# hsiehScalAR/KNODE-Cosserat

Hardware: AMD Instinct MI355X
Metric: rod-steps/sec (N=100 segments, batch=1024) (higher is better)
Workload: dtype f64

## Files before the change

knode-cosserat_amd/csrc/kr_mso_impl.hpp:

```cpp
#pragma once
#include "kr_ms_impl.hpp"

namespace kr {

constexpr int MSO_B0 = 7 + 17 * (MS_P - 1);
#ifndef KR_MSO_LAG
#define KR_MSO_LAG 1
#endif
constexpr int MSO_LAG = KR_MSO_LAG;
#ifndef KR_MSO_TRIP_WAITS
#define KR_MSO_TRIP_WAITS 1
#endif
#ifndef KR_MSO_TRIP_CARRY
#define KR_MSO_TRIP_CARRY 0
#endif
static_assert(MSO_B0 + MS_P <= WAVE, "the verifying lanes must fit beside the forward-difference lanes");

template <typename T, int HS>
__host__ __device__ inline size_t mso_lds_elems(int N) {
  return ms_lds_elems<T, HS>(N, true, false) + 80;
}

__device__ __forceinline__ void wave_sync_lds() {
  __builtin_amdgcn_fence(__ATOMIC_ACQ_REL, "wavefront");
  __builtin_amdgcn_wave_barrier();
}

#define KR_LDS __attribute__((address_space(3)))
#define KR_SCHED_ALL_BUT_DS 0x047f
template <typename T, int NV>
__device__ __forceinline__ void lds_load_vec(const T* src, T (&v)[NV]) {
  using V = typename Vec16<T>::type;
  constexpr int n = Vec16<T>::n;
  static_assert(NV % n == 0, "vector load needs a multiple of 16 bytes");
  const KR_LDS V* s = (const KR_LDS V*)src;
#pragma unroll
  for (int c = 0; c < NV / n; ++c) {
    const V x = s[c];
#pragma unroll
    for (int e = 0; e < n; ++e) v[c * n + e] = x[e];
  }
}
template <typename T, int NV>
__device__ __forceinline__ void lds_store_vec(T* dst, const T (&v)[NV]) {
  using V = typename Vec16<T>::type;
  constexpr int n = Vec16<T>::n;
  static_assert(NV % n == 0, "vector store needs a multiple of 16 bytes");
  KR_LDS V* d = (KR_LDS V*)dst;
#pragma unroll
  for (int c = 0; c < NV / n; ++c) {
    V x;
#pragma unroll
    for (int e = 0; e < n; ++e) x[e] = v[c * n + e];
    d[c] = x;
  }
}

template <typename T>
struct LeadTile {
  using V = typename Vec16<T>::type;
  static constexpr int NT = 12 / Vec16<T>::n;
  V t[NT];
};
template <typename T>
__device__ __forceinline__ void lds_load_lead(const T* src, LeadTile<T>& x) {
  using V = typename Vec16<T>::type;
  const KR_LDS V* s = (const KR_LDS V*)src;
#pragma unroll
  for (int c = 0; c < LeadTile<T>::NT; ++c) x.t[c] = s[c];
}
__device__ __forceinline__ void lead_pin(LeadTile<double>& x) {
  asm volatile("" : "+v"(x.t[0]), "+v"(x.t[1]), "+v"(x.t[2]), "+v"(x.t[3]), "+v"(x.t[4]), "+v"(x.t[5]));
}
template <typename T>
__device__ __forceinline__ void lead_unpack(const LeadTile<T>& x, T (&v)[12]) {
  constexpr int n = Vec16<T>::n;
#pragma unroll
  for (int c = 0; c < LeadTile<T>::NT; ++c) {
#pragma unroll
    for (int e = 0; e < n; ++e) v[c * n + e] = x.t[c][e];
  }
}

template <typename U>
__device__ __forceinline__ U own_sgpr(U v) {
  asm volatile("" : "+s"(v));
  return v;
}

template <typename U>
__device__ __forceinline__ U* own_sgpr_global(U* p) {
  uintptr_t v = (uintptr_t)p;
  asm volatile("" : "+s"(v));
  return (U*)(__attribute__((address_space(1))) U*)v;
}

template <typename T>
__device__ __forceinline__ T quad_pick(int kp, T v0, T v1, T v2, T v3) {
  T v = v3;
  v = kp == 2 ? v2 : v;
  v = kp == 1 ? v1 : v;
  v = kp == 0 ? v0 : v;
  return v;
}

template <int K>
__device__ __forceinline__ void wave_sum_f64_staged(double (&v)[K]) {
  auto stage = [&](auto ctrl) {
    double o[K];
#pragma unroll
    for (int k = 0; k < K; ++k) o[k] = quad_xor<decltype(ctrl)::value>(v[k]);
#pragma unroll
    for (int k = 0; k < K; ++k) v[k] += o[k];
  };
  stage(std::integral_constant<int, 0xB1>{});
  stage(std::integral_constant<int, 0x4E>{});
  stage(std::integral_constant<int, 0x141>{});
  stage(std::integral_constant<int, 0x140>{});
  int lo[K], hi[K];
  double s[K];
#pragma unroll
  for (int k = 0; k < K; ++k) {
    const long long b = __double_as_longlong(v[k]);
    lo[k] = (int)(b & 0xFFFFFFFFll);
    hi[k] = (int)(b >> 32);
    s[k] = 0.0;
  }
#pragma unroll
  for (int r = 0; r < 4; ++r) {
#pragma unroll
    for (int k = 0; k < K; ++k) {
      const int l = __builtin_amdgcn_readlane(lo[k], 16 * r), h = __builtin_amdgcn_readlane(hi[k], 16 * r);
      s[k] += __longlong_as_double(((long long)h << 32) | (unsigned int)l);
    }
  }
#pragma unroll
  for (int k = 0; k < K; ++k) v[k] = s[k];
}

template <typename T, int NC>
__device__ __forceinline__ void mso_pred_update(MsPred<T, NC>& Q, int order, int predictor, int lane, const T* Xs,
                                                MsStamps& stamps) {
  if (!__builtin_amdgcn_readfirstlane((int)(order == MS_ORDER_LP && Q.lp_good))) {
    ms_pred_update<T>(Q, order, KR_ST_CONVERGED, predictor, lane, Xs, stamps);
    return;
  }
#ifdef KR_MS_STAMPS
  unsigned long long tpu;
  KR_STAMP(tpu);
#endif
  float err_lp = 0.f;
  if (Q.lp_have) {
#pragma unroll
    for (int q = 0; q < MS_EPL; ++q) {
      const int e = lane + q * WAVE;
      if (e < MS_NE) {
        const double x = (double)Xs[e];
        double b[NC];
        lp_basis<T, NC>(Q.Hx[q], b);
        err_lp = fmaxf(err_lp, update_ratio(x - lp_eval<NC>(Q.lpa, b), x));
      }
    }
  }
  const float em_lp = wave_max_nonneg(err_lp);
#ifdef KR_MS_STAMPS
  KR_STAMP_ADD(stamps.a1, tpu);
#endif
  const bool lp_tested = Q.lp_have;
  const bool keep_fit = lp_tested && em_lp < 1.0e-3f && Q.lp_age < 3;
  Q.lp_age = keep_fit ? Q.lp_age + 1 : 0;
  Q.lp_have = keep_fit;
  if (!keep_fit && predictor >= MS_ORDER_LP && Q.avail >= NC - 1) {
    double Sn[lp_nsum<NC>()];
#pragma unroll
    for (int k = 0; k < lp_nsum<NC>(); ++k) Sn[k] = 0.0;
#pragma unroll
    for (int q = 0; q < MS_EPL; ++q) {
      const int e = lane + q * WAVE;
      if (e < MS_NE) {
        const double x = (double)Xs[e];
        double b[NC];
        lp_basis<T, NC>(Q.Hx[q], b);
        const double w = (double)__builtin_amdgcn_rcpf(fmaxf(fabsf((float)x), 1.0f));
        lp_accumulate<NC>(Sn, b, x, w);
      }
    }
    if constexpr (sizeof(T) == 8) {
      wave_sum_f64_staged(Sn);
    } else {
#pragma unroll
      for (int k = 0; k < lp_nsum<NC>(); ++k) Sn[k] = wave_sum_f64(Sn[k]);
    }
    double a[NC];
    if (lp_solve<NC>(Sn, a)) {
#pragma unroll
      for (int k = 0; k < NC; ++k) Q.lpa[k] = a[k];
      Q.lp_have = true;
    }
  }
#ifdef KR_MS_STAMPS
  KR_STAMP_ADD(stamps.a2, tpu);
#endif
  Q.next_order = Q.avail < predictor ? Q.avail : (predictor < MS_HLEV ? predictor : MS_HLEV - 1);
  Q.lp_good = lp_tested && Q.lp_have && em_lp < 1.0e-3f;
  if (lp_tested && Q.lp_have && (em_lp < 3.0e38f || Q.lp_good)) Q.next_order = MS_ORDER_LP;
#ifdef KR_MS_STAMPS
  stamps.osum += (unsigned long long)order; stamps.olast = order;
  for (int p = 0; p < MS_HLEV; ++p) stamps.em[p] = 3.0e38f;
  KR_STAMP_ADD(stamps.a3, tpu);
#endif
#pragma unroll
  for (int q = 0; q < MS_EPL; ++q) {
    const int e = lane + q * WAVE;
#pragma unroll
    for (int k = MS_HLEV - 1; k > 0; --k) Q.Hx[q][k] = Q.Hx[q][k - 1];
    if (e < MS_NE) Q.Hx[q][0] = Xs[e];
  }
  if (Q.avail < MS_HLEV - 1) ++Q.avail;
}

#ifdef KR_MS_STAMPS
struct MsoStats { unsigned long long total = 0, sweeps = 0, merged = 0, quick = 0, chord = 0, rejects = 0, retries = 0, rebuilds = 0, t_sweep = 0, t_alg = 0, t_pred = 0, t_verdict = 0, t_cond = 0, t_fin = 0, t_upd = 0, t_v1 = 0, t_v2 = 0, t_c1 = 0, t_c2 = 0, t_copy = 0; };
#endif

template <typename T, bool DIAG, int HS, int OCC = 1, typename PSRC = RodConst<T>>
__global__ __launch_bounds__(WAVE * MS_WPB, OCC) void mso_sim_kernel(const PSRC Pa, const SimArgs<T> A) {
  extern __shared__ __attribute__((aligned(16))) unsigned char smem_raw[];
  const int N = rod_src_N<T>(Pa);
  const int lane = threadIdx.x & (WAVE - 1);
  const int wv = threadIdx.x / WAVE;
  const int64_t rod = (int64_t)blockIdx.x * MS_WPB + wv;
  if (rod >= A.B) return;
  const auto& Pc = rod_src_row<T>(Pa, rod);
  const size_t rod_elems = (size_t)N * KR_SLOTS;
  T* const a_states = own_sgpr_global(A.states);
  const int64_t a_slot_elems = own_sgpr(A.slot_elems);
  const int a_ring = own_sgpr(A.ring);
  T* const a_tip = own_sgpr_global(A.tip);
  int32_t* const a_status = own_sgpr_global(A.status);
  const int a_residual_test = own_sgpr(A.residual_test), a_predictor = own_sgpr(A.predictor);
  const T hc1 = own_sgpr(A.hc1), hc2 = own_sgpr(A.hc2);
  const int T_steps = own_sgpr((int)A.T_steps);
  using KPSRC = rod_src_keypoints<T, PSRC>;
  constexpr bool KP = KPSRC::value;
  constexpr bool TRIM = OCC == 1 && sizeof(T) == 8 && MSO_LAG == 1;
  const unsigned long long kp_lo = KPSRC::lo(Pa), kp_hi = KPSRC::hi(Pa);
  const MsLds<T> L = ms_carve<T, HS>(reinterpret_cast<T*>(smem_raw) + (size_t)wv * mso_lds_elems<T, HS>(N), N, true, false);
  T* const Es = L.Es;
  T* const XB = L.XB;
  T* const Tm = L.Tm;
  T* const X0 = L.Xs;
  const ptrdiff_t X_d = (L.c12 + (size_t)N * 12) - L.Xs;
  int xsel = 0;
  T* Xs = X0;
  T* XsB = X0 + X_d;
  T* const EsB = Es + MSO_B0 * MS_YP;
  const MsRole R = ms_role(lane, N);
  const int iv = R.iv, col = R.col;
  const bool isA = lane < MSO_B0;
  const bool isB = lane >= MSO_B0 && lane < MSO_B0 + MS_P;
  const int ib = isB ? lane - MSO_B0 : 0;
  const int s_l = isB ? ms_interval_start(ib, R.sbase, R.srem) : R.s_i;
  const int len_l = isB ? R.sbase + (ib < R.srem ? 1 : 0) : R.len_i;
  unsigned kp_marks = 0;
  int kp_rank0 = 0;
  if constexpr (KP) {
    kp_marks = keypoint_window(kp_lo, kp_hi, s_l);
    kp_rank0 = keypoint_rank(kp_lo, kp_hi, s_l);
  }
  ms_cold_fill<T>(rod_src_mem<T>(Pa, rod), L.cold, lane);
  wave_sync();

  auto slot_ptr = [&](int slot) -> T* { return a_states + (int64_t)slot * a_slot_elems + rod * rod_elems; };
  auto state_ptr = [&](int k) -> T* { return slot_ptr(a_ring ? k % 3 : k); };
  T* const lead0 = L.c12;
  const ptrdiff_t lead_d = L.hist - L.c12;
  auto lead_of = [&](int t) -> T* { return lead0 + (ptrdiff_t)(t & 1) * lead_d; };
  auto rebuild = [&](int t) {
    const T* cur = state_ptr(t);
    const T* prv = t > 0 ? state_ptr(t - 1) : (A.prev_init ? A.prev_init + rod * rod_elems : cur);
    T* const lc = lead_of(t);
    T* const lp = lead_of(t - 1);
    for (int j = lane; j < N; j += WAVE) {
      T cv[12], pv[12];
      load_hist_vec<T, 12>(cur + (size_t)j * KR_SLOTS, cv);
      load_hist_vec<T, 12>(prv + (size_t)j * KR_SLOTS, pv);
      lds_store_vec<T, 12>(lc + (size_t)j * 12, cv);
      lds_store_vec<T, 12>(lp + (size_t)j * 12, pv);
    }
    wave_sync();
  };
  using WSRC = rod_src_step_slots<T, PSRC>;
  constexpr int W0 = WSRC::first, WN = WSRC::count;
  constexpr bool LOADS = WN > 0;
  static_assert(!LOADS || (W0 + WN == CD_TDIRS && (W0 == CD_FTIP || W0 == CD_P0)), "the per-step slots end with F_tip, M_tip");
  static_assert(!LOADS || (HS >= 18 && (2 * MS_P + 1) * (HS - 12) >= WN), "the second set lives behind the odd tile in the record area");
  const ptrdiff_t wr_d = LOADS ? (L.hist + (size_t)N * 12) - (L.cold + W0) : 0;
  auto cold_of = [&](int t) -> const T* {
    if constexpr (LOADS) return L.cold + (ptrdiff_t)(t & 1) * wr_d;
    else return L.cold;
  };
  auto base_of = [&](int t) -> const T* {
    if constexpr (LOADS && W0 < CD_FTIP) return L.cold + (ptrdiff_t)(t & 1) * wr_d;
    else return L.cold;
  };
  const T* wrench = nullptr;
  if constexpr (LOADS) wrench = WSRC::hist(Pa) + rod * A.T_steps * WN;
  const T* ctl = A.ctl + rod * A.T_steps * 4;
  auto load_fc = [&](int t) -> V3<T> {
    V3<T> tf{T(0), T(0), T(0)};
#pragma unroll
    for (int k = 0; k < 4; ++k) {
      const T tt = ctl[(size_t)t * 4 + k];
      tf.x += tt * L.cold[CD_TDIRS + k * 3 + 0];
      tf.y += tt * L.cold[CD_TDIRS + k * 3 + 1];
      tf.z += tt * L.cold[CD_TDIRS + k * 3 + 2];
    }
    return {L.cold[CD_RHOAG] + tf.x, L.cold[CD_RHOAG + 1] + tf.y, L.cold[CD_RHOAG + 2] + tf.z};
  };

  const T* s0 = state_ptr(0);
  const T* sp0 = A.prev_init ? A.prev_init + rod * rod_elems : s0;
  MsPred<T> Q;
  double* img = A.pred_io ? A.pred_io + (size_t)rod * MS_PRED_ROWS * WAVE : nullptr;
  if (img && A.pred_load) ms_pred_load<T>(Q, img, lane);
  else ms_pred_init<T>(Q, lane, R, s0, sp0, A.prev_init != nullptr, a_predictor);
  V3<T> vlast, ulast;
  {
    const T* cl = s0 + (size_t)(N - 1) * KR_SLOTS;
    vlast = {cl[SL_V], cl[SL_V + 1], cl[SL_V + 2]};
    ulast = {cl[SL_U], cl[SL_U + 1], cl[SL_U + 2]};
  }
  const T tol = own_sgpr(A.tol), tolA = own_sgpr(A.tolA), fd_eps = own_sgpr(A.fd_eps);
  const int maxit = own_sgpr(A.maxit);
  T kappa = Q.kappa;
  T Gguess = lane < 6 ? A.G[rod * 6 + lane] : T(0);
  MsStamps stamps;
#ifdef KR_MS_STAMPS
  MsoStats st;
  unsigned long long t_begin, tq;
  KR_STAMP(t_begin);
  tq = t_begin;
#endif

  rebuild(0);

  int tA = 0;
  int rsA = 0;
  bool merged = false;
  int it = 0;
  int order = Q.next_order;
  bool retried = false;
  T dn_prev = T(-1);
  bool have_fac = false, below = false;
  float amp = -1.f;
  T dnB = T(-1);
  float ampB = -1.f;
  bool belowB = false;
  int itB = 0, orderB = 0;
  bool pred_skip = false;
  bool reverify = false;
  int resume_at = T_steps;
  T Xreg[MS_P - 1][2];
#pragma unroll
  for (int g = 0; g < MS_P - 1; ++g) Xreg[g][0] = Xreg[g][1] = T(0);
  V3<T> fcA = load_fc(0), fcB = fcA;
  V3<T> fcN = load_fc(T_steps > 1 ? 1 : 0);
  T wN = T(0);
  if constexpr (LOADS) {
    if (lane < WN) {
      L.cold[W0 + lane] = wrench[lane];
      wN = wrench[(size_t)(T_steps > 1 ? 1 : 0) * WN + lane];
    }
    if constexpr (W0 < CD_FTIP) wave_sync_lds();
  }
  static_assert(DIAG, "the in-sweep history record assumes diagonal material matrices");
  T hk_a[3], hk_b[3], hk_c[3];
#pragma unroll
  for (int c = 0; c < 3; ++c) {
    hk_a[c] = L.cold[CD_KSEI + 4 * c] * L.cold[CD_KSEV + c];
    hk_b[c] = -L.cold[CD_KSEI + 4 * c] * L.cold[CD_BSE + 4 * c];
    hk_c[c] = -L.cold[CD_KBTI + 4 * c] * L.cold[CD_BBT + 4 * c];
  }

  ms_pred_guess<T>(Q, order, lane, base_of(0), Xs);
  wave_sync_lds();
  if (order <= 0 && lane < 6) Xs[0 * MS_YP + 7 + lane] = Gguess;
  wave_sync_lds();

  struct Upd { T newPG, newY[MS_P - 1]; };

  while (true) {
    const bool runA = tA < T_steps;
    const int tB = tA - 1;
    T yr[19];
    {
      const T* src = isB ? XsB + ib * MS_YP : Xs + iv * MS_YP;
#pragma unroll
      for (int q = 0; q < 19; ++q) yr[q] = src[q];
    }
    const T hstep = (isA && col > 0) ? fd_eps * fmax(fabs(Xs[iv * MS_YP + (R.comp > 0 ? R.comp : 3)]), T(1)) : T(1);
    int comp = R.comp;
    asm volatile("" : "+v"(comp));
#pragma unroll
    for (int q = 3; q < 19; ++q) yr[q] += q == comp ? hstep : T(0);
    RodState<T> y = rows_to_state(yr);
    const V3<T> fc = isB ? fcB : fcA;
    const int lag = (isA && merged) ? MSO_LAG : 0;
    const bool act = isB ? merged : (isA && runA);
    const int trips = R.lmax + ((merged && runA) ? MSO_LAG : 0);
    T* const out_rod = slot_ptr(rsA);
    T* const kp_out = KPSRC::at(Pa, tB, A.B, rod);
    auto point_of = [&](int k) -> int {
      const int kk = k - lag;
      return s_l + (kk < 0 ? 0 : (kk < len_l ? kk : len_l - 1));
    };
    const T* const lead_n = lead_of(isB ? tB : tA);
    const T* const lead_o = lead_of(isB ? tB + 1 : tB);
    auto hist_older = [&](const T (&lb)[12], T (&pb)[12]) __attribute__((always_inline)) {
#pragma unroll
      for (int c = 0; c < 12; ++c) pb[c] = hc2 * lb[c];
    };
    auto hist_newest = [&](const T (&la)[12], const T (&pb)[12]) __attribute__((always_inline)) -> RodHist<T> {
      T raw[12];
#pragma unroll
      for (int c = 0; c < 12; ++c) raw[c] = fma(hc1, la[c], pb[c]);
      RodHist<T> h;
      h.qh = {raw[0], raw[1], raw[2]};
      h.wh = {raw[3], raw[4], raw[5]};
      h.vh = {raw[6], raw[7], raw[8]};
      h.uh = {raw[9], raw[10], raw[11]};
      h.av = {hk_b[0] * raw[6] + hk_a[0], hk_b[1] * raw[7] + hk_a[1], hk_b[2] * raw[8] + hk_a[2]};
      h.au = {hk_c[0] * raw[9], hk_c[1] * raw[10], hk_c[2] * raw[11]};
      return h;
    };
    auto hist_form = [&](const T (&la)[12], const T (&lb)[12]) __attribute__((always_inline)) -> RodHist<T> {
      T pb[12];
      hist_older(lb, pb);
      return hist_newest(la, pb);
    };
    auto hist_at = [&](int j) __attribute__((always_inline)) -> RodHist<T> {
      T la[12], lb[12];
      lds_load_vec<T, 12>(lead_n + (size_t)j * 12, la);
      lds_load_vec<T, 12>(lead_o + (size_t)j * 12, lb);
      return hist_form(la, lb);
    };
    RodHist<T> hst = hist_at(point_of(0));
    const bool lean = a_ring && tB + 4 <= T_steps;
    if (!merged) {
      auto fd_point = [&](int j, T dsl) __attribute__((always_inline)) {
        RodState<T> k1;
        V3<T> v, u;
        ode_eval<T, DIAG>(Pc, y, hst, fc, k1, v, u);
        hst = hist_at(j + 1);
        y = state_axpy(y, dsl, k1);
      };
#pragma unroll 2
      for (int t = 0; t < R.sbase; ++t) fd_point(R.s_i + t, Pc.ds);
      if (R.srem) fd_point(R.s_i + (R.len_i > R.sbase ? R.sbase : R.sbase - 1), R.len_i > R.sbase ? Pc.ds : T(0));
    } else {
      T* const lead_w = lead_of(tB + 1);
#if KR_MSO_TRIP_CARRY
      T rs = rot_scale(y.h0, y.h1, y.h2, y.h3);
#endif
      auto trip = [&](int k, auto full_tag, auto lean_tag) __attribute__((always_inline)) {
        constexpr int FORM = decltype(full_tag)::value;
        constexpr bool FULL = FORM == 1;
        constexpr bool FIRST = TRIM && FORM == 2;
        constexpr bool LEAN = decltype(lean_tag)::value;
        const int kk = k - lag;
        const bool live = FIRST ? isB : FULL ? act : (act && kk >= 0 && kk < len_l);
        const int j = FIRST ? s_l : FULL ? s_l + kk : point_of(k);
        const int eo = j * 12;
        const int en = FIRST ? (s_l + ((isB && len_l > 1) ? 1 : 0)) * 12 : FULL ? eo + 12 : point_of(k + 1) * 12;
        T la[12], lb[12], pb[12];
#ifdef KR_MSO_PROBE_EARLY_READS
        constexpr bool TUPLES = false;
#else
        constexpr bool TUPLES = KR_MSO_TRIP_WAITS && MSO_LAG < 2 && OCC == 1 && sizeof(T) == 8;
#endif
        LeadTile<T> ta, tb;
        if constexpr (TUPLES) {
          lds_load_lead<T>(lead_o + en, tb);
          __builtin_amdgcn_sched_barrier(KR_SCHED_ALL_BUT_DS);
        } else if constexpr (MSO_LAG >= 2) {
          lds_load_vec<T, 12>(lead_n + en, la);
          lds_load_vec<T, 12>(lead_o + en, lb);
        } else {
          lds_load_vec<T, 12>(lead_o + en, lb);
#ifdef KR_MSO_PROBE_EARLY_READS
          if constexpr (FULL) lds_load_vec<T, 12>(lead_n + en, la);
#endif
        }
        RodState<T> k1;
        V3<T> v, u;
#if KR_MSO_TRIP_CARRY
        ode_eval_s<T, DIAG>(Pc, y, hst, fc, k1, v, u, rs);
#else
        ode_eval<T, DIAG>(Pc, y, hst, fc, k1, v, u);
#endif
        if constexpr (MSO_LAG >= 2) {
          hst = hist_form(la, lb);
          asm volatile("" : "+v"(hst.qh.x), "+v"(hst.qh.y), "+v"(hst.qh.z), "+v"(hst.wh.x), "+v"(hst.wh.y), "+v"(hst.wh.z));
          asm volatile("" : "+v"(hst.vh.x), "+v"(hst.vh.y), "+v"(hst.vh.z), "+v"(hst.uh.x), "+v"(hst.uh.y), "+v"(hst.uh.z));
          asm volatile("" : "+v"(hst.av.x), "+v"(hst.av.y), "+v"(hst.av.z), "+v"(hst.au.x), "+v"(hst.au.y), "+v"(hst.au.z));
        } else {
          if constexpr (TUPLES) {
            asm volatile("" ::"v"(v.x), "v"(v.y), "v"(v.z), "v"(u.x), "v"(u.y), "v"(u.z));
            lead_pin(tb);
            lead_unpack<T>(tb, lb);
          }
          hist_older(lb, pb);
          asm volatile("" : "+v"(pb[0]), "+v"(pb[1]), "+v"(pb[2]), "+v"(pb[3]), "+v"(pb[4]), "+v"(pb[5]), "+v"(pb[6]), "+v"(pb[7]),
                            "+v"(pb[8]), "+v"(pb[9]), "+v"(pb[10]), "+v"(pb[11]));
        }
        if (isB && live) {
          T rec[KR_SLOTS];
          record_from(y, v, u, rec);
          T lead[12];
#pragma unroll
          for (int c = 0; c < 12; ++c) lead[c] = rec[c];
          if constexpr (FULL) {
            if constexpr (!LEAN) {
              T rest[KR_SLOTS - 12];
#pragma unroll
              for (int c = 0; c < KR_SLOTS - 12; ++c) rest[c] = rec[12 + c];
              store_vec<T, KR_SLOTS - 12>(out_rod + (size_t)j * KR_SLOTS + 12, rest);
            }
          } else {
            if (!(lean && k >= R.sbase)) store_record(out_rod + (size_t)j * KR_SLOTS, rec);
          }
          if constexpr (KP) store_keypoint_window(kp_out, kp_marks, kp_rank0, kk, rec);
#ifdef KR_MSO_PROBE_NO_TILE_STORES
          if constexpr (!FULL)
#endif
#ifdef KR_MSO_PROBE_ONE_TILE_STORE
          if constexpr (FULL) {
            T l2[Vec16<T>::n];
#pragma unroll
            for (int c = 0; c < Vec16<T>::n; ++c) l2[c] = lead[c];
            lds_store_vec<T, Vec16<T>::n>(lead_w + eo, l2);
          } else
#endif
          lds_store_vec<T, 12>(lead_w + eo, lead);
        }
        if constexpr (MSO_LAG < 2) {
#ifdef KR_MSO_PROBE_EARLY_READS
          if constexpr (!FULL)
#endif
          {
            if constexpr (TUPLES) lds_load_lead<T>(lead_n + en, ta);
            else lds_load_vec<T, 12>(lead_n + en, la);
          }
          if constexpr (OCC == 1) __builtin_amdgcn_sched_barrier(0);
        }
        const T dsl = live ? Pc.ds : T(0);
        y = state_axpy(y, dsl, k1);
        if constexpr (MSO_LAG < 2) {
          asm volatile("" : "+v"(pb[0]), "+v"(pb[1]), "+v"(pb[2]), "+v"(pb[3]), "+v"(pb[4]), "+v"(pb[5]), "+v"(pb[6]), "+v"(pb[7]),
                            "+v"(pb[8]), "+v"(pb[9]), "+v"(pb[10]), "+v"(pb[11]), "+v"(y.p.z), "+v"(y.h3), "+v"(y.n.z), "+v"(y.m.z),
                            "+v"(y.q.z), "+v"(y.w.z));
#if KR_MSO_TRIP_CARRY
          rs = rot_scale(y.h0, y.h1, y.h2, y.h3);
#endif
          if constexpr (TUPLES) {
            lead_pin(ta);
            lead_unpack<T>(ta, la);
          }
          hst = hist_newest(la, pb);
        }
      };
      int k = 0;
      for (; k < MSO_LAG && k < trips; ++k) trip(k, std::integral_constant<int, 2>{}, std::false_type{});
      auto full_trips = [&](auto lean_tag) __attribute__((always_inline)) {
        for (; k + 1 < R.sbase; k += 2) {
          trip(k, std::true_type{}, lean_tag);
          trip(k + 1, std::true_type{}, lean_tag);
        }
        if (k < R.sbase) {
          trip(k, std::true_type{}, lean_tag);
          ++k;
        }
      };
      if (lean) full_trips(std::true_type{});
      else full_trips(std::false_type{});
      const bool own_final = TRIM && runA;
      for (; k < trips - (own_final ? 1 : 0); ++k) trip(k, std::false_type{}, std::false_type{});
      if (own_final) {
        const bool live = isA && R.lmax - 1 < len_l;
        RodState<T> k1;
        V3<T> v, u;
        ode_eval<T, DIAG>(Pc, y, hst, fc, k1, v, u);
        const T dsl = live ? Pc.ds : T(0);
        y = state_axpy(y, dsl, k1);
      }
    }
#ifdef KR_MS_STAMPS
    KR_STAMP_ADD(st.t_sweep, tq);
    st.sweeps += 1;
    if (merged) st.merged += 1;
#endif

    int ln = lane;
    asm volatile("" : "+v"(ln));
    const int kp = ln & 3;
    const int r = 3 + (ln >> 2);
    const bool plane = ln < 3 * (MS_P - 1);
    const int pi = plane ? ln / 3 : 0;
    const int prow = plane ? ln - 3 * pi : 0;
    const bool glane = ln >= WAVE - 6;
    T er[19];
    state_to_rows(y, er);
    T d[6];
    T updY[MS_P - 1];
    T* dYb = XB;
    float dnf = 0.f;
    bool finite = true;
    Upd U;

    auto finish = [&](const T* X, auto base_slot) -> float {
      T* sp = Tm;
      if (kp == 0) {
#pragma unroll
        for (int g = 1; g < MS_P - 1; ++g) dYb[g * MS_YP + r] = updY[g - 1];
      }
      wave_sync_lds();
      if (plane) {
        const bool p0 = pi == 0;
        const int l0 = p0 ? 0 : 7 + 17 * (pi - 1);
        const int drow = p0 ? 1 : pi;
        T s = Es[base_slot(pi) * MS_YP + prow] - X[(pi + 1) * MS_YP + prow];
        T av[16], dv[16];
#pragma unroll
        for (int c = 0; c < 16; ++c) {
          av[c] = Es[(l0 + 1 + c) * MS_YP + prow];
          dv[c] = dYb[drow * MS_YP + 3 + c];
        }
        __builtin_amdgcn_sched_barrier(0);
        T s2 = T(0);
#pragma unroll
        for (int c = 0; c < 6; c += 2) {
          s = fma(av[c], p0 ? d[c] : dv[c], s);
          s2 = fma(av[c + 1], p0 ? d[c + 1] : dv[c + 1], s2);
        }
        const T s_6 = s, s2_6 = s2;
#pragma unroll
        for (int c = 6; c < 16; c += 2) {
          s = fma(av[c], dv[c], s);
          s2 = fma(av[c + 1], dv[c + 1], s2);
        }
        s = p0 ? s_6 : s;
        s2 = p0 ? s2_6 : s2;
        sp[pi * 3 + prow] = s + s2;
      }
      wave_sync_lds();
      const T xp = X[(pi + 1) * MS_YP + prow];
      T up = T(0);
#pragma unroll
      for (int i = 0; i < MS_P - 1; ++i) {
        const T t = sp[i * 3 + prow];
        up += i <= pi ? t : T(0);
      }
      const int kg = glane ? ln - (WAVE - 6) : 0;
      const T xg = X[0 * MS_YP + 7 + kg];
      T ug = d[5];
      asm volatile("" : "+v"(ug));
      ug = kg == 4 ? d[4] : ug;
      ug = kg == 3 ? d[3] : ug;
      asm volatile("" : "+v"(ug));
      ug = kg == 2 ? d[2] : ug;
      ug = kg == 1 ? d[1] : ug;
      asm volatile("" : "+v"(ug));
      ug = kg == 0 ? d[0] : ug;
      const T newP = xp + up, newG = xg + ug;
      U.newPG = plane ? newP : newG;
      float np = update_ratio(up, xp), ng = update_ratio(ug, xg);
      asm volatile("" : "+v"(np), "+v"(ng));
      unsigned nb = plane ? __float_as_uint(np) : (glane ? __float_as_uint(ng) : 0u);
#pragma unroll
      for (int g = 1; g < MS_P; ++g) {
        const T xy = X[g * MS_YP + r];
        float ny = update_ratio(updY[g - 1], xy);
        U.newY[g - 1] = xy + updY[g - 1];
        asm volatile("" : "+v"(ny));
        nb = max(nb, ((g - 1) & 3) == kp ? __float_as_uint(ny) : 0u);
      }
      const float nf = __uint_as_float(nb);
      return wave_max_nonneg(nf);
    };
    auto apply = [&](T* X) {
      int la = ln;
      asm volatile("" : "+v"(la));
      const bool pl = la < 3 * (MS_P - 1), gl = la >= WAVE - 6;
      const int pa = pl ? la / 3 : 0;
      if (pl || gl) X[pl ? (pa + 1) * MS_YP + (la - 3 * pa) : 0 * MS_YP + 7 + (la - (WAVE - 6))] = U.newPG;
#pragma unroll
      for (int g = 1; g < MS_P; ++g)
        if (g - 1 == (la & 3)) X[g * MS_YP + r] = U.newY[g - 1];
    };

    const bool es_stored = merged;
    if (merged) {
      if (isB || (isA && col == 0)) {
#pragma unroll
        for (int q = 0; q < 19; ++q) Es[ln * MS_YP + q] = er[q];
      }
      if (isB) {
        if (ib == MS_P - 1) {
          T rec[KR_SLOTS];
          record_from(y, vlast, ulast, rec);
          if (!lean) store_record(out_rod + (size_t)(N - 1) * KR_SLOTS, rec);
          if constexpr (KP) store_keypoint(kp_out, kp_lo, kp_hi, N - 1, rec);
          T lead[12];
#pragma unroll
          for (int c = 0; c < 12; ++c) lead[c] = rec[c];
          lds_store_vec<T, 12>(lead_of(tB + 1) + (size_t)(N - 1) * 12, lead);
          if (a_tip) {
            T* tp = a_tip + (rod * T_steps + tB) * 3;
            tp[0] = y.p.x; tp[1] = y.p.y; tp[2] = y.p.z;
          }
        }
      }
      wave_sync_lds();
#ifdef KR_MS_STAMPS
      unsigned long long tv;
      { KR_STAMP(tv); st.t_v1 += tv - tq; }
#endif
      float rn = 0.f;
      if (ln < 3 * MS_YP) {
        const int g = ln / MS_YP, q = ln - MS_YP * g;
        const T x = XsB[(g + 1) * MS_YP + q];
        rn = update_ratio(EsB[g * MS_YP + q] - x, x);
      } else if (ln < 3 * MS_YP + 6) {
        const int k = ln - 3 * MS_YP;
        const T e = EsB[(MS_P - 1) * MS_YP + 7 + k];
        rn = update_ratio(cold_of(tB)[CD_FTIP + k] - e, e);
      }
      rn = wave_max_nonneg(rn);
#ifdef KR_MS_STAMPS
      KR_STAMP_ADD(st.t_v2, tv);
#endif
      const float est = ampB * rn;
      bool accepted = a_residual_test != 0 && ampB > 0.f && T(256) * (T)est <= tol;
      float dnv = est;
#ifdef KR_MS_STAMPS
      if (accepted) st.quick += 1;
#endif
      if (!accepted) {
        T* ach = XB;
        T* rt = XB + 4 * MS_YP;
        dYb = XB + MS_YP * 8;
        T areg[MS_P - 1];
        areg[0] = EsB[0 * MS_YP + r] - XsB[1 * MS_YP + r];
        constexpr bool HOP = TRIM;
        if constexpr (!HOP) {
          if (kp == 0) ach[1 * MS_YP + r] = areg[0];
          wave_sync_lds();
        }
#pragma unroll
        for (int g = 1; g < MS_P; ++g) {
          const int l0 = 7 + 17 * (g - 1);
          T av[4], xv[4];
#pragma unroll
          for (int cc = 0; cc < 4; ++cc) {
            av[cc] = Es[(l0 + 1 + 4 * kp + cc) * MS_YP + r];
            if (HOP && g == 1) xv[cc] = EsB[0 * MS_YP + 3 + 4 * kp + cc] - XsB[1 * MS_YP + 3 + 4 * kp + cc];
            else xv[cc] = ach[g * MS_YP + 3 + 4 * kp + cc];
          }
          const T e0 = EsB[g * MS_YP + r];
          const T ynext = g < MS_P - 1 ? XsB[(g + 1) * MS_YP + r] : T(0);
          T part = fma(av[0], xv[0], av[1] * xv[1]) + fma(av[2], xv[2], av[3] * xv[3]);
          part += quad_xor<0xB1>(part);
          part += quad_xor<0x4E>(part);
          if (g < MS_P - 1) {
            areg[g] = e0 - ynext + part;
            if (kp == 0) ach[(g + 1) * MS_YP + r] = areg[g];
          } else if (kp == 0 && r >= 7 && r < 13) {
            rt[r - 7] = cold_of(tB)[CD_FTIP + (r - 7)] - e0 - part;
          }
          wave_sync_lds();
        }
        if constexpr (HOP) {
          const int di = ln < 6 ? ln : 0;
          T acc = T(0);
#pragma unroll
          for (int j = 0; j < 6; ++j) acc = fma(L.Ti[di * 6 + j], rt[j], acc);
          d[0] = lane_bcast<0>(acc); d[1] = lane_bcast<1>(acc); d[2] = lane_bcast<2>(acc);
          d[3] = lane_bcast<3>(acc); d[4] = lane_bcast<4>(acc); d[5] = lane_bcast<5>(acc);
        } else {
          T rtv[6];
#pragma unroll
          for (int j = 0; j < 6; ++j) rtv[j] = rt[j];
#pragma unroll
          for (int i = 0; i < 6; ++i) {
            T acc = T(0);
#pragma unroll
            for (int j = 0; j < 6; ++j) acc = fma(L.Ti[i * 6 + j], rtv[j], acc);
            d[i] = acc;
          }
        }
        {
          const T dd0 = quad_pick<T>(kp, T(0), d[1], d[3], d[5]);
          const T dd1 = quad_pick<T>(kp, d[0], d[2], d[4], T(0));
#pragma unroll
          for (int g = 1; g < MS_P; ++g) {
            T sx = fma(Xreg[g - 1][1], dd1, Xreg[g - 1][0] * dd0);
            sx += quad_xor<0xB1>(sx);
            sx += quad_xor<0x4E>(sx);
            updY[g - 1] = areg[g - 1] + sx;
          }
        }
        dnv = finish(XsB, [](int g) { return MSO_B0 + g; });
        accepted = dnv <= 3.0e38f && (T)dnv <= T(0.5) * tol;
#ifdef KR_MS_STAMPS
        st.chord += 1;
#endif
      }
      if (accepted) {
        {
          const T* const lt = lead_of(tB + 1);
          for (int j = ln; j < N; j += WAVE) {
            T lv[12];
            lds_load_vec<T, 12>(lt + (size_t)j * 12, lv);
            store_vec<T, 12>(out_rod + (size_t)j * KR_SLOTS, lv);
          }
        }
        if (!belowB && dnB > T(0)) {
          const T floor_dn = T(64) * (sizeof(T) == 8 ? T(2.2e-16) : T(1.2e-7));
          const T kq = fmax((T)dnv, floor_dn) * fast_rcp(dnB * dnB);
          kappa = fmin(fmax(kq, T(1e-4)), T(1));
        }
        if (ln == 0 && a_status) a_status[rod * T_steps + tB] = KR_ST_CONVERGED;
        if (ln < 6) Gguess = XsB[0 * MS_YP + 7 + ln];
        pred_skip = false;
        reverify = false;
        merged = false;
        if (!runA) break;
      } else {
#ifdef KR_MS_STAMPS
        st.rejects += 1;
#endif
        const bool ok = dnv <= 3.0e38f;
        if (ok) apply(XsB);
        wave_sync_lds();
        if (ok && !reverify && itB + 2 <= maxit) {
          reverify = true;
          itB += 1;
          dnB = (T)dnv;
          __builtin_amdgcn_fence(__ATOMIC_ACQ_REL, "agent");
          rebuild(tB);
#ifdef KR_MS_STAMPS
          st.rebuilds += 1;
          KR_STAMP_ADD(st.t_alg, tq);
#endif
          continue;
        }
        reverify = false;
        for (int e = ln; e < MS_NE; e += WAVE) Xs[e] = XsB[e];
        tA = tB;
        rsA = a_ring ? (rsA == 0 ? 2 : rsA - 1) : rsA - 1;
        fcN = fcA;
        fcA = fcB;
        if constexpr (LOADS) {
          if (lane < WN) wN = wrench[(size_t)(tA + 1 < T_steps ? tA + 1 : tA) * WN + lane];
        }
        order = orderB;
        it = itB;
        dn_prev = ok ? (T)dnv : T(-1);
        have_fac = ok;
        amp = ampB;
        below = false;
        pred_skip = true;
        merged = false;
        __builtin_amdgcn_fence(__ATOMIC_ACQ_REL, "agent");
        rebuild(tA);
#ifdef KR_MS_STAMPS
        st.rebuilds += 1;
        KR_STAMP_ADD(st.t_alg, tq);
#endif
        if (it >= maxit) { resume_at = tA; break; }
        continue;
      }
    }

#ifdef KR_MS_STAMPS
    { unsigned long long t_; KR_STAMP(t_); st.t_verdict += t_ - tq; }
    unsigned long long tq2;
    KR_STAMP(tq2);
#endif
    ++it;
    float res_full;
    {
      const int l0own = iv == 0 ? 0 : 7 + 17 * (iv - 1);
      if (!es_stored) {
        if (isA && col == 0) {
#pragma unroll
          for (int q = 0; q < 19; ++q) Es[ln * MS_YP + q] = er[q];
        }
        wave_sync_lds();
      }
      res_full = ms_residual_norm<T>(Es, Xs, cold_of(tA), ln);
      if (isA && col > 0) {
        const T ih = fast_rcp(hstep);
        T e0[19];
#pragma unroll
        for (int q = 0; q < 19; ++q) e0[q] = Es[l0own * MS_YP + q];
        __builtin_amdgcn_sched_barrier(0);
#pragma unroll
        for (int q = 0; q < 19; ++q) Es[ln * MS_YP + q] = (er[q] - e0[q]) * ih;
      }
      wave_sync_lds();
    }
#ifdef KR_MS_STAMPS
    unsigned long long tc;
    { KR_STAMP(tc); st.t_c1 += tc - tq2; }
#endif
    dYb = XB;
    {
      const T c0 = Es[0 * MS_YP + r] - Xs[1 * MS_YP + r];
      const T da = Es[(2 * kp) * MS_YP + r];
      const T db = Es[(2 * kp + 1) * MS_YP + r];
      Xreg[0][0] = kp == 0 ? c0 : da;
      Xreg[0][1] = kp == 3 ? T(0) : db;
      store_pair(XB + r * 8 + 2 * kp, Xreg[0][0], Xreg[0][1]);
    }
    wave_sync_lds();
#pragma unroll
    for (int g = 1; g < MS_P; ++g) {
      const T* xcur = XB + ((g - 1) & 1) * (MS_YP * 8);
      T* xnext = XB + (g & 1) * (MS_YP * 8);
      const int l0 = 7 + 17 * (g - 1);
      const T e0 = Es[l0 * MS_YP + r];
      T n0 = T(0), n1 = T(0), n2 = T(0), n3 = T(0);
      if (g < MS_P - 1) {
        const T cg = e0 - Xs[(g + 1) * MS_YP + r];
        n0 = kp == 0 ? cg : T(0);
      }
      {
        T av[16], xa[16], xb[16];
#pragma unroll
        for (int c = 0; c < 16; ++c) {
          av[c] = Es[(l0 + 1 + c) * MS_YP + r];
          load_pair(xcur + (3 + c) * 8 + 2 * kp, xa[c], xb[c]);
        }
        __builtin_amdgcn_sched_barrier(0);
#pragma unroll
        for (int c = 0; c < 16; c += 2) {
          n0 = fma(av[c], xa[c], n0);
          n1 = fma(av[c], xb[c], n1);
          n2 = fma(av[c + 1], xa[c + 1], n2);
          n3 = fma(av[c + 1], xb[c + 1], n3);
        }
        n0 += n2;
        n1 += n3;
      }
      if (g < MS_P - 1) {
        Xreg[g][0] = n0;
        Xreg[g][1] = n1;
        store_pair(xnext + r * 8 + 2 * kp, n0, n1);
      } else if (r >= 7 && r < 13) {
        if (kp == 0) n0 = cold_of(tA)[CD_FTIP + (r - 7)] - e0 - n0;
        store_pair(Tm + (r - 7) * 8 + 2 * kp, n0, n1);
      }
      wave_sync_lds();
    }
#ifdef KR_MS_STAMPS
    KR_STAMP_ADD(st.t_c2, tc);
#endif
    {
      T a6[6][7];
      auto fill6 = [&](T (&m)[6][7]) {
#pragma unroll
        for (int i = 0; i < 6; ++i) {
          T row[8];
          load_hist_vec<T, 8>(Tm + i * 8, row);
#pragma unroll
          for (int k = 0; k < 6; ++k) m[i][k] = row[1 + k];
          m[i][6] = ln < 6 ? (ln == i ? T(1) : T(0)) : row[0];
        }
      };
      fill6(a6);
      T x6[6];
      solve6_uniform(a6, x6, fill6);
      if (ln < 6) {
#pragma unroll
        for (int i = 0; i < 6; ++i) L.Ti[i * 6 + ln] = x6[i];
      }
#pragma unroll
      for (int i = 0; i < 6; ++i) d[i] = lane_bcast<6>(x6[i]);
      have_fac = true;
    }
    {
      const T dd0 = quad_pick<T>(kp, T(1), d[1], d[3], d[5]);
      const T dd1 = quad_pick<T>(kp, d[0], d[2], d[4], T(0));
#pragma unroll
      for (int g = 1; g < MS_P; ++g) {
        T s = fma(Xreg[g - 1][1], dd1, Xreg[g - 1][0] * dd0);
        s += quad_xor<0xB1>(s);
        s += quad_xor<0x4E>(s);
        updY[g - 1] = s;
      }
    }
#ifdef KR_MS_STAMPS
    KR_STAMP_ADD(st.t_cond, tq2);
#endif
    dnf = finish(Xs, [](int g) { return g == 0 ? 0 : 7 + 17 * (g - 1); });
#ifdef KR_MS_STAMPS
    KR_STAMP_ADD(st.t_fin, tq2);
#endif
    finite = dnf <= 3.0e38f;
    const T dn = (T)dnf;
    if (res_full > 0.f && finite) amp = dnf / res_full;
    if (finite && !below && dn <= tol) {
      below = true;
      if (dn_prev > T(0)) {
        const T floor_dn = T(64) * (sizeof(T) == 8 ? T(2.2e-16) : T(1.2e-7));
        const T kq = fmax(dn, floor_dn) * fast_rcp(dn_prev * dn_prev);
        kappa = fmin(fmax(kq, T(1e-4)), T(1));
      }
    }
    bool next_final = false;
    if (finite) {
      apply(Xs);
      next_final = predict_final<T>(dn, dn_prev, tol, tolA) || (kappa > T(0) && T(4) * kappa * dn * dn <= tol);
      dn_prev = dn;
    }
    wave_sync_lds();
#ifdef KR_MS_STAMPS
    KR_STAMP_ADD(st.t_alg, tq);
#endif
    if (!finite || (it >= maxit && !(next_final && dn <= T(1e-2)))) {
      if (order > 0 && !retried) {
        retried = true;
        order = 0;
        ms_pred_guess<T>(Q, 0, ln, base_of(tA), Xs);
        wave_sync_lds();
        if (ln < 6) Xs[0 * MS_YP + 7 + ln] = Gguess;
        wave_sync_lds();
        it = 0; dn_prev = T(-1); have_fac = false; amp = -1.f; below = false;
#ifdef KR_MS_STAMPS
        st.retries += 1;
#endif
        continue;
      }
      resume_at = tA;
      break;
    }
    if (next_final && dn <= T(1e-2)) {
      xsel ^= 1;
      Xs = X0 + xsel * X_d;
      XsB = X0 + (1 - xsel) * X_d;
#ifdef KR_MS_STAMPS
      { unsigned long long t_; KR_STAMP(t_); st.t_copy += t_ - tq; }
#endif
      dnB = dn; ampB = amp; belowB = below; itB = it; orderB = order;
      if (!pred_skip) {
        if constexpr (OCC == 1) mso_pred_update<T>(Q, order, a_predictor, lane, XsB, stamps);
        else ms_pred_update<T>(Q, order, KR_ST_CONVERGED, a_predictor, lane, XsB, stamps);
      }
#ifdef KR_MS_STAMPS
      { unsigned long long t_; KR_STAMP(t_); st.t_upd += t_ - tq; }
#endif
      tA += 1;
      rsA = a_ring ? (rsA == 2 ? 0 : rsA + 1) : rsA + 1;
      fcB = fcA;
      if (tA < T_steps) {
        fcA = fcN;
        fcN = load_fc(tA + 1 < T_steps ? tA + 1 : tA);
        if constexpr (LOADS) {
          if (lane < WN) {
            L.cold[W0 + wr_d * (tA & 1) + lane] = wN;
            wN = wrench[(size_t)(tA + 1 < T_steps ? tA + 1 : tA) * WN + lane];
          }
          if constexpr (W0 < CD_FTIP) wave_sync_lds();
        }
        order = Q.next_order;
        ms_pred_guess<T>(Q, order, lane, base_of(tA), Xs);
        wave_sync_lds();
        if (order <= 0 && lane < 6) Xs[0 * MS_YP + 7 + lane] = XsB[0 * MS_YP + 7 + lane];
        wave_sync_lds();
      }
      it = 0; retried = false; below = false; dn_prev = T(-1);
      merged = true;
#ifdef KR_MS_STAMPS
      KR_STAMP_ADD(st.t_pred, tq);
#endif
    }
  }

  if (lane < 6) A.G[rod * 6 + lane] = Gguess;
  if (lane == 0 && A.resume) A.resume[rod] = (int32_t)resume_at;
  if (img && (resume_at >= T_steps || !A.resume)) {
    Q.kappa = kappa;
    ms_pred_save<T>(Q, img, lane);
  }
#ifdef KR_MS_STAMPS
  if (lane == 0 && A.dbg) {
    unsigned long long te;
    KR_STAMP(te);
    unsigned long long* dd = A.dbg + rod * 24;
    dd[0] = te - t_begin; dd[1] = st.t_sweep; dd[2] = st.t_alg; dd[3] = st.t_pred; dd[4] = st.sweeps;
    dd[5] = st.merged; dd[6] = st.quick; dd[7] = st.chord; dd[8] = st.rejects; dd[9] = st.retries; dd[10] = st.rebuilds;
    dd[11] = (unsigned long long)resume_at;
    dd[12] = st.t_verdict; dd[13] = st.t_cond; dd[14] = st.t_fin; dd[15] = st.t_upd;
    dd[16] = stamps.a1; dd[17] = stamps.a2; dd[18] = stamps.a3; dd[19] = st.t_v1; dd[20] = st.t_v2; dd[21] = st.t_c1; dd[22] = st.t_c2; dd[23] = st.t_copy;
  }
#endif
}

template <typename T, int OCC, typename PSRC>
static int launch_mso_inst(const PSRC& P, const SimPlan& p, const SimArgs<T>& a, const LaunchAt& at) {
  return launch(at, mso_sim_kernel<T, true, hs_phys<T>(), OCC, PSRC>, dim3((unsigned)((a.B + MS_WPB - 1) / MS_WPB)), dim3(WAVE * MS_WPB),
                p.smem[0], P, a);
}
template <typename T>
int launch_mso_sim(kr_handle* h, const SimPlan& p, const SimArgs<T>& a, const LaunchAt& at) {
  if constexpr (sizeof(T) == 4) {
    if (p.occ == 2) return launch_mso_inst<T, 2>(consts<T>(h), p, a, at);
  }
  return launch_mso_inst<T, 1>(consts<T>(h), p, a, at);
}

}
```

Baseline: 49.64 million.

## Park accepted lead tile in registers instead of rebuilding from global on reject

Keeps a register copy of the lead state tile taken when a step is accepted. On a rejected step, the tile is restored from registers rather than fenced and reloaded from global memory. In lean mode it also skips writing each accepted tile to global memory, and instead writes the current and previous tiles out once at exit when the solve stops early. This trades higher register pressure (MS_NPL x 12 doubles per lane) for fewer global round trips and fewer agent-scope fences.

```diff
diff --git a/knode-cosserat_amd/csrc/kr_mso_impl.hpp b/knode-cosserat_amd/csrc/kr_mso_impl.hpp
--- a/knode-cosserat_amd/csrc/kr_mso_impl.hpp
+++ b/knode-cosserat_amd/csrc/kr_mso_impl.hpp
@@ -8,6 +8,9 @@
 #define KR_MSO_LAG 1
 #endif
 constexpr int MSO_LAG = KR_MSO_LAG;
+#ifndef KR_MSO_PARK
+#define KR_MSO_PARK 1
+#endif
 #ifndef KR_MSO_TRIP_WAITS
 #define KR_MSO_TRIP_WAITS 1
 #endif
@@ -217,6 +220,27 @@
     if (e < MS_NE) Q.Hx[q][0] = Xs[e];
   }
   if (Q.avail < MS_HLEV - 1) ++Q.avail;
+}
+
+template <typename T>
+struct MsoPark { T v[MS_NPL][12]; };
+struct MsoNoPark { };
+template <typename T>
+__device__ __forceinline__ void mso_park_take(MsoPark<T>& park, const T* lt, int lane, int N) {
+#pragma unroll
+  for (int q = 0; q < MS_NPL; ++q) {
+    const int j = lane + q * WAVE;
+    lds_load_vec<T, 12>(lt + (size_t)(j < N ? j : N - 1) * 12, park.v[q]);
+  }
+}
+template <typename T>
+__device__ __forceinline__ void mso_park_restore(const MsoPark<T>& park, T* lt, int lane, int N) {
+#pragma unroll
+  for (int q = 0; q < MS_NPL; ++q) {
+    const int j = lane + q * WAVE;
+    if (j < N) lds_store_vec<T, 12>(lt + (size_t)j * 12, park.v[q]);
+  }
+  wave_sync_lds();
 }
 
 #ifdef KR_MS_STAMPS
@@ -244,6 +268,7 @@
   using KPSRC = rod_src_keypoints<T, PSRC>;
   constexpr bool KP = KPSRC::value;
   constexpr bool TRIM = OCC == 1 && sizeof(T) == 8 && MSO_LAG == 1;
+  constexpr bool PARK = TRIM && KR_MSO_PARK != 0;
   const unsigned long long kp_lo = KPSRC::lo(Pa), kp_hi = KPSRC::hi(Pa);
   const MsLds<T> L = ms_carve<T, HS>(reinterpret_cast<T*>(smem_raw) + (size_t)wv * mso_lds_elems<T, HS>(N), N, true, false);
   T* const Es = L.Es;
@@ -290,6 +315,15 @@
     }
     wave_sync();
   };
+  std::conditional_t<PARK, MsoPark<T>, MsoNoPark> park;
+  static_assert(!PARK || MS_NPL * WAVE >= 128, "the park holds every grid point the planner serves (one_wave_range)");
+  if constexpr (PARK) {
+#pragma unroll
+    for (int q = 0; q < MS_NPL; ++q) {
+#pragma unroll
+      for (int c = 0; c < 12; ++c) park.v[q][c] = T(0);
+    }
+  }
   using WSRC = rod_src_step_slots<T, PSRC>;
   constexpr int W0 = WSRC::first, WN = WSRC::count;
   constexpr bool LOADS = WN > 0;
@@ -817,7 +851,13 @@
 #endif
       }
       if (accepted) {
-        {
+        bool tile_pass = true;
+#ifdef KR_MSO_PROBE_NO_TILE_PASS
+        tile_pass = !lean;
+#else
+        if constexpr (PARK) tile_pass = !lean;
+#endif
+        if (tile_pass) {
           const T* const lt = lead_of(tB + 1);
           for (int j = ln; j < N; j += WAVE) {
             T lv[12];
@@ -847,8 +887,12 @@
           reverify = true;
           itB += 1;
           dnB = (T)dnv;
-          __builtin_amdgcn_fence(__ATOMIC_ACQ_REL, "agent");
-          rebuild(tB);
+          if constexpr (PARK) {
+            mso_park_restore<T>(park, lead_of(tB + 1), lane, N);
+          } else {
+            __builtin_amdgcn_fence(__ATOMIC_ACQ_REL, "agent");
+            rebuild(tB);
+          }
 #ifdef KR_MS_STAMPS
           st.rebuilds += 1;
           KR_STAMP_ADD(st.t_alg, tq);
@@ -872,8 +916,12 @@
         below = false;
         pred_skip = true;
         merged = false;
-        __builtin_amdgcn_fence(__ATOMIC_ACQ_REL, "agent");
-        rebuild(tA);
+        if constexpr (PARK) {
+          mso_park_restore<T>(park, lead_of(tA + 1), lane, N);
+        } else {
+          __builtin_amdgcn_fence(__ATOMIC_ACQ_REL, "agent");
+          rebuild(tA);
+        }
 #ifdef KR_MS_STAMPS
         st.rebuilds += 1;
         KR_STAMP_ADD(st.t_alg, tq);
@@ -1054,6 +1102,7 @@
       { unsigned long long t_; KR_STAMP(t_); st.t_copy += t_ - tq; }
 #endif
       dnB = dn; ampB = amp; belowB = below; itB = it; orderB = order;
+      if constexpr (PARK) mso_park_take<T>(park, lead_of(tA + 1), lane, N);
       if (!pred_skip) {
         if constexpr (OCC == 1) mso_pred_update<T>(Q, order, a_predictor, lane, XsB, stamps);
         else ms_pred_update<T>(Q, order, KR_ST_CONVERGED, a_predictor, lane, XsB, stamps);
@@ -1088,6 +1137,23 @@
     }
   }
 
+  if constexpr (PARK) {
+    if (resume_at < T_steps) {
+      const T* const lc = lead_of(resume_at);
+      const T* const lp = lead_of(resume_at - 1);
+      T* const oc = state_ptr(resume_at);
+      T* const op = resume_at > 0 ? state_ptr(resume_at - 1) : nullptr;
+      for (int j = lane; j < N; j += WAVE) {
+        T lv[12];
+        lds_load_vec<T, 12>(lc + (size_t)j * 12, lv);
+        store_vec<T, 12>(oc + (size_t)j * KR_SLOTS, lv);
+        if (op) {
+          lds_load_vec<T, 12>(lp + (size_t)j * 12, lv);
+          store_vec<T, 12>(op + (size_t)j * KR_SLOTS, lv);
+        }
+      }
+    }
+  }
   if (lane < 6) A.G[rod * 6 + lane] = Gguess;
   if (lane == 0 && A.resume) A.resume[rod] = (int32_t)resume_at;
   if (img && (resume_at >= T_steps || !A.resume)) {
```

After: 50.67 million, median of 6. 2.1% higher.
